# piotrkawa/audio-deepfake-adversarial-attacks

Measured on AMD Instinct MI355X. Metric: adversarial utterances/sec, PGD-40 LCNN+LFCC 4s@16kHz, higher is better.
Workload: dtype f32

## Files before the change

### audio_deepfake_adversarial_attacks_amd/csrc/lfcc_stft.hip

```cpp

#include <hip/hip_runtime.h>
#include <math.h>
#include <stdint.h>
#include <stdlib.h>

#include "advstep_frontend.h"
#include "advstep_common.h"
#include "stft_reg.h"

namespace {

constexpr int kWavesPerBlock = 4;
constexpr int kThreads = kWavesPerBlock * 64;
constexpr int kFramesPerBlockBwd = 4;
static_assert(kFramesPerBlockBwd == kGroup, "overlap_add_frames (stft_reg.h) sums the frames of one group");

__device__ __forceinline__ float2 cmul(float2 a, float2 b) { return make_float2(a.x * b.x - a.y * b.y, a.x * b.y + a.y * b.x); }

__device__ __forceinline__ void wave_lds_sync() {
    __builtin_amdgcn_fence(__ATOMIC_RELEASE, "workgroup");
    __builtin_amdgcn_wave_barrier();
    __builtin_amdgcn_fence(__ATOMIC_ACQUIRE, "workgroup");
}

// ... 132 lines not shown
    __syncthreads();
    if (threadIdx.x == 0) {
        float r = L.red[0];
        for (int i = 1; i < kWavesPerBlock; ++i) r = max_nan(r, L.red[i]);
        bmax[b * gridDim.x + blockIdx.x] = r;
    }
}

constexpr int kMaxSpanT = 8, kMaxBands = 128;

__device__ __forceinline__ void frame_spectrum(const float *__restrict__ xb, const float *__restrict__ w, int T, int f,
                                               int hop, Lds &L, int wave, int lane) {
    load_frame(xb, w, T, f, hop, L.a[wave], lane);
    wave_lds_sync();
    fft256<false>(L.a[wave], L.b[wave], L.tw, lane);
    unpack_real(L.a[wave], L.tw512, L.xs_of(wave), lane);
    wave_lds_sync();
}

__device__ __forceinline__ float2 one_sided_scale(float2 gk, int k) {
    if (k == 0 || k == kN) gk.y = 0.0f;
    else gk.x *= 0.5f, gk.y *= 0.5f;
    return gk;
}

template <bool PRESCALED>
__device__ __forceinline__ void spectrum_grad_to_frame(Lds &L, int wave, int lane, const float *__restrict__ w, float *dst,
                                                       bool live) {
    if (!PRESCALED) {
        for (int k = lane; k < kBins; k += 64) L.xs_of(wave)[k] = one_sided_scale(L.xs_of(wave)[k], k);
        wave_lds_sync();
    }
    for (int k = lane; k < kN; k += 64) {
        const float2 gk = L.xs_of(wave)[k], gc = conjf2(L.xs_of(wave)[kN - k]);
        const float2 e = cadd(gk, gc), d = csub(gk, gc);
        const float2 wd = cmul(conjf2(L.tw512[k]), d);
        L.a[wave][P(k)] = make_float2(e.x - wd.y, e.y + wd.x);
    }
    wave_lds_sync();
    fft256<true>(L.a[wave], L.b[wave], L.tw, lane);
    for (int n = lane; n < kN; n += 64) {
        const float2 z = L.a[wave][P(n)];
        const float2 wv = reinterpret_cast<const float2 *>(w)[n];
        reinterpret_cast<float2 *>(dst)[n] = live ? make_float2(wv.x * z.x, wv.y * z.y) : make_float2(0.0f, 0.0f);
    }
    wave_lds_sync();
}

template <int STRIDE>
__device__ __attribute__((noinline)) void overlap_add_frames_cold(const float *dframe, float *__restrict__ dxb, int f_base, int NF, int hop,
                                                                  int T, int tid, int nthreads);

__device__ __forceinline__ void overlap_add_block(const float (*dframe)[kNfft], float *__restrict__ dxb, int f_base, int NF,
                                                  int hop, int T) {
    overlap_add_frames<kNfft>(&dframe[0][0], dxb, f_base, NF, hop, T, threadIdx.x, kThreads);
}

template <int STRIDE>
__device__ __attribute__((noinline)) void overlap_add_frames_cold(const float *dframe, float *__restrict__ dxb, int f_base, int NF, int hop,
                                                                  int T, int tid, int nthreads) {
    overlap_add_frames<STRIDE>(dframe, dxb, f_base, NF, hop, T, tid, nthreads);
}

template <int SPAN_CAP>
struct LdsBwd {
    Lds c;
    float dframe[kFramesPerBlockBwd][kNfft];
    float fbt_w[kBins * SPAN_CAP];
    int32_t fbt_start[kBins];
    float drow[kWavesPerBlock][kMaxBands];
};

template <int SPAN_CAP>
__global__ __launch_bounds__(kThreads) void stft_bands_backward_kernel(const float *__restrict__ x,
                                                                       const float *__restrict__ w,
                                                                       const float *__restrict__ dband,
                                                                       const int32_t *__restrict__ fbt_start,
                                                                       const float *__restrict__ fbt_w, int span_t,
                                                                       float *__restrict__ dx, int T, int NF, int hop,
                                                                       int M) {
    extern __shared__ __attribute__((aligned(16))) unsigned char raw[];
    LdsBwd<SPAN_CAP> &S = *reinterpret_cast<LdsBwd<SPAN_CAP> *>(raw);
    Lds &L = S.c;
    {
        static_assert(kN == kThreads, "one twiddle pair per thread");
        constexpr int kWIt = (kBins * SPAN_CAP + kThreads - 1) / kThreads;
        const int m = threadIdx.x, nw = kBins * span_t;
        const float2 t0 = stage_twiddle(m < kStageTw ? m : 0), t1 = kTw512[m];
        const int32_t s0 = fbt_start[m], s1 = fbt_start[kThreads + (m < kBins - kThreads ? m : 0)];
        float wq[kWIt];
#pragma unroll
        for (int j = 0; j < kWIt; ++j) {
            const int i = m + j * kThreads;
            wq[j] = fbt_w[i < nw ? i : nw - 1];
        }
        if (m < kStageTw) L.tw[m] = t0;
        L.tw512[m] = t1;
        S.fbt_start[m] = s0;
        if (m < kBins - kThreads) S.fbt_start[kThreads + m] = s1;
#pragma unroll
        for (int j = 0; j < kWIt; ++j) {
            const int i = m + j * kThreads;
            if (i < nw) S.fbt_w[i] = wq[j];
        }
    }
    __syncthreads();
    const int wave = threadIdx.x >> 6, lane = threadIdx.x & 63;
    const int64_t b = blockIdx.y;
    const int f_base = blockIdx.x * kFramesPerBlockBwd;
    const float *xb = x + b * T;
    for (int r = 0; r < kFramesPerBlockBwd / kWavesPerBlock; ++r) {
        const int fl = r * kWavesPerBlock + wave;
        const int f = f_base + fl;
        const bool live = f < NF;
        const float *drow_g = dband + (b * NF + (live ? f : NF - 1)) * M;
        for (int m = lane; m < M; m += 64) S.drow[wave][m] = drow_g[m];
        load_frame(xb, w, T, live ? f : NF - 1, hop, L.a[wave], lane);
        wave_lds_sync();
        fft256<false>(L.a[wave], L.b[wave], L.tw, lane);
        const float *drow = S.drow[wave];
        auto grad_of_bin = [&](int k, float2 xk) {
            const int m0 = S.fbt_start[k];
            float dp = 0.0f;
            for (int j = 0; j < span_t; ++j) {
                const int m = m0 + j;
                if (m < M) dp = fmaf(S.fbt_w[k * span_t + j], drow[m], dp);
            }
            return one_sided_scale(make_float2(2.0f * xk.x * dp, 2.0f * xk.y * dp), k);
        };
        {
            const float2 *Z = L.a[wave];
            for (int k = lane; k < kN; k += 64) {
                const float2 zk = Z[P(k)], zc = conjf2(Z[P((kN - k) & (kN - 1))]);
                const float2 e = make_float2(0.5f * (zk.x + zc.x), 0.5f * (zk.y + zc.y));
                const float2 d = make_float2(0.5f * (zk.x - zc.x), 0.5f * (zk.y - zc.y));
                const float2 o = cmul(L.tw512[k], make_float2(d.y, -d.x));
                L.xs_of(wave)[k] = grad_of_bin(k, cadd(e, o));
            }
            if (lane == 0) L.xs_of(wave)[kN] = grad_of_bin(kN, make_float2(Z[P(0)].x - Z[P(0)].y, 0.0f));
        }
        wave_lds_sync();
        spectrum_grad_to_frame<true>(L, wave, lane, w, S.dframe[fl], live);
    }
    __syncthreads();
    overlap_add_block(S.dframe, dx + b * T, f_base, NF, hop, T);
}

#ifndef STFT_FWD_GROUPS
#define STFT_FWD_GROUPS 2
#endif
constexpr int kGroupsPerWave = STFT_FWD_GROUPS;
constexpr int kBandsFramesPerBlock = kWavesPerBlock * kGroupsPerWave * kGroup;

struct LdsReg {
    float2 blk[kWavesPerBlock][kGroup][kFrameSlots];
    float2 twl[16 * kPitch];
    float red[kWavesPerBlock];
};

__device__ __forceinline__ void fill_reg_tables(LdsReg &S) {
    for (int m = threadIdx.x; m < kN; m += kThreads) S.twl[(m >> 4) * kPitch + (m & 15)] = kTw256[((m >> 4) * (m & 15)) & 255];
}

__device__ __forceinline__ void load_frame_reg(const float *__restrict__ xb, const float2 *__restrict__ win2, int T, int f, int hop,
                                               float2 (&x)[16], int l) {
    const int q_first = f * hop - kN;
    if (q_first >= 0 && q_first + kNfft <= T && ((q_first & 1) == 0) && ((reinterpret_cast<uintptr_t>(xb) & 7u) == 0)) {
        const float2 *x2 = reinterpret_cast<const float2 *>(xb + q_first);
        float2 v[16];
#pragma unroll
        for (int r = 0; r < 16; ++r) v[r] = x2[16 * r + l];
#pragma unroll
        for (int r = 0; r < 16; ++r) {
            const float2 wv = win2[16 * r + l];
            x[r] = make_float2(wv.x * v[r].x, wv.y * v[r].y);
        }
        return;
    }
#pragma unroll
    for (int r = 0; r < 16; ++r) {
        const int n = 16 * r + l;
        int q0 = q_first + 2 * n, q1 = q0 + 1;
        q0 = q0 < 0 ? -q0 : q0;
        q0 = q0 >= T ? 2 * (T - 1) - q0 : q0;
        q1 = q1 < 0 ? -q1 : q1;
        q1 = q1 >= T ? 2 * (T - 1) - q1 : q1;
        const float2 wv = win2[n];
        x[r] = make_float2(wv.x * xb[q0], wv.y * xb[q1]);
    }
}

constexpr int kRegSpan = 4;

struct LdsRegFwd {
    LdsReg c;
    float fbw[kMaxBands * kRegSpan];
    int32_t fbs[kMaxBands];
};

__global__ __launch_bounds__(kThreads) void stft_bands_reg_kernel(const float *__restrict__ x, const float *__restrict__ w,
                                                                  const int32_t *__restrict__ fb_start,
                                                                  const float *__restrict__ fb_w, int span,
                                                                  float *__restrict__ band_db, float *__restrict__ bmax, int T,
                                                                  int NF, int hop, int M, int bmax_tail) {
    __shared__ LdsRegFwd SF;
    LdsReg &S = SF.c;
    fill_reg_tables(S);
    for (int i = threadIdx.x; i < kMaxBands * kRegSpan; i += kThreads) {
        const int m = i / kRegSpan, j = i % kRegSpan;
        SF.fbw[i] = (m < M && j < span) ? 0.25f * fb_w[m * span + j] : 0.0f;
    }
    for (int m = threadIdx.x; m < kMaxBands; m += kThreads) SF.fbs[m] = m < M ? fb_start[m] : 0;
    const int wave = threadIdx.x >> 6, lane = threadIdx.x & 63, fs = lane >> 4, l = lane & 15;
    __syncthreads();
    const int64_t b = blockIdx.y;
    float2 *blk = S.blk[wave][fs];
    float vmax = -INFINITY;
    for (int g = 0; g < kGroupsPerWave; ++g) {
        const int f0 = blockIdx.x * kBandsFramesPerBlock + (wave * kGroupsPerWave + g) * kGroup;
        if (f0 >= NF) break;
        const int f = f0 + fs;
        const bool live = f < NF;
        float2 xr[16];
        load_frame_reg(x + b * T, reinterpret_cast<const float2 *>(w), T, live ? f : NF - 1, hop, xr, here(l));
        fft256_reg<false>(xr, S.twl, blk, l);
        float nyq;
        unpack_real_reg(xr, nyq, blk, l);
        phase_done(xr);
        float *pw = reinterpret_cast<float *>(blk);
        lds_wave_fence();
#pragma unroll
        for (int r = 0; r < 16; ++r) pw[l + 16 * r] = fmaf(xr[r].x, xr[r].x, xr[r].y * xr[r].y);
        if (l == 0) pw[kN] = nyq * nyq;
        if (l >= 1 && l <= kRegSpan) pw[kN + l] = 0.0f;
        lds_wave_fence();
        float *row = band_db + (b * NF + (live ? f : NF - 1)) * M;
#pragma unroll
        for (int half = 0; half < 2; ++half) {
            int k0[4];
            float wt[4][kRegSpan], pv[4][kRegSpan];
#pragma unroll
            for (int i = 0; i < 4; ++i) k0[i] = SF.fbs[l + 16 * (4 * half + i)];
#pragma unroll
            for (int i = 0; i < 4; ++i)
#pragma unroll
                for (int j = 0; j < kRegSpan; ++j) {
                    wt[i][j] = SF.fbw[(l + 16 * (4 * half + i)) * kRegSpan + j];
                    pv[i][j] = pw[k0[i] + j];
                }
#pragma unroll
            for (int i = 0; i < 4; ++i) {
                const int m = l + 16 * (4 * half + i);
                float band = 0.0f;
#pragma unroll
                for (int j = 0; j < kRegSpan; ++j) band = fmaf(wt[i][j], pv[i][j], band);
                const float db = 3.010299956639812f * __log2f(band > kAmin ? band : (band != band ? band : kAmin));
                if (live && m < M) {
                    row[m] = db;
                    vmax = max_nan(vmax, db);
                }
            }
        }
        lds_wave_fence();
    }
    vmax = wave_reduce(vmax, MaxNanOp());
    if (lane == 0) S.red[wave] = vmax;
    __syncthreads();
    if (threadIdx.x == 0) {
        float r = S.red[0];
        for (int i = 1; i < kWavesPerBlock; ++i) r = max_nan(r, S.red[i]);
        bmax[b * gridDim.x + blockIdx.x] = r;
        const int total = gridDim.x * gridDim.y;
        for (int j = (int)b * gridDim.x + blockIdx.x; j < bmax_tail; j += total) bmax[total + j] = -INFINITY;
    }
}

template <int STRIDE>
__device__ __forceinline__ void overlap_add_interior(const float *df, float *__restrict__ out, int lane, float (&carry)[6],
                                                     bool carry_in, bool carry_out) {
    constexpr int HOP = 160, kSpan = 3 * HOP + kNfft, kShared = kNfft - HOP;
    static_assert(4 * HOP == 640 && kSpan <= 16 * 64, "slices");
#pragma unroll
    for (int j = 0; j < 16; ++j) {
        if (j % 4 == 0) lds_wave_fence();
        float acc = 0.0f;
#pragma unroll
        for (int fl = 0; fl < 4; ++fl) {
            const int lo = HOP * fl - 64 * j, hi = lo + kNfft;
            if (hi <= 0 || lo >= 64) continue;
            if (lo <= 0 && hi >= 64) {
                acc += df[fl * STRIDE + lane - lo];
            } else {
                const int n = lane - lo;
                if ((unsigned)n < (unsigned)kNfft) acc += df[fl * STRIDE + n];
            }
        }
        const int i = lane + 64 * j;
        if (j < 6) {
            const bool shared = i < kShared;
            if (carry_in) {
                out[i] = shared ? acc + carry[j] : acc;
            } else if (j < 5) {
                atomicAdd(out + i, acc);
            } else {
                if (shared) atomicAdd(out + i, acc);
                else out[i] = acc;
            }
        } else if (j < 10) {
            out[i] = acc;
        } else {
            if (carry_out) carry[j - 10] = acc;
            else if (i < kSpan) atomicAdd(out + i, acc);
        }
    }
}

template <int SPAN_CAP>
struct LdsRegBwd {
    LdsReg c;
    float fbt_w[(kBins + 1) * SPAN_CAP];
    int32_t fbt_start[kBins + 1];
};

#ifndef STFT_BWD_GROUPS
#define STFT_BWD_GROUPS 4
#endif
constexpr int kBwdGroupsPerWave = STFT_BWD_GROUPS;
constexpr int kBwdFramesPerBlock = kWavesPerBlock * kBwdGroupsPerWave * kGroup;

#ifndef STFT_BWD_WAVES
#define STFT_BWD_WAVES 4
#endif
template <int SPAN_CAP>
__global__ __launch_bounds__(kThreads) __attribute__((amdgpu_waves_per_eu(STFT_BWD_WAVES, STFT_BWD_WAVES)))
void stft_bands_backward_reg_kernel(const float *__restrict__ x,
                                                                           const float *__restrict__ w,
                                                                           const float *__restrict__ dband,
                                                                           const int32_t *__restrict__ fbt_start,
                                                                           const float *__restrict__ fbt_w, int span_t,
                                                                           float *__restrict__ dx, int T, int NF, int hop,
                                                                           int M, const float *__restrict__ band_db,
                                                                           const float *__restrict__ stats) {
    extern __shared__ __attribute__((aligned(16))) unsigned char raw[];
    LdsRegBwd<SPAN_CAP> &S = *reinterpret_cast<LdsRegBwd<SPAN_CAP> *>(raw);
    float fix_share = 0.0f, fix_max = 0.0f;
    bool fix = false;
    if (stats != nullptr) {
        const float s2 = stats[2];
        if (s2 != 0.0f) {
            fix = true;
            fix_max = stats[0];
            fix_share = s2 / (stats[1] > 0.0f ? stats[1] : 1.0f);
        }
    }
    fill_reg_tables(S.c);
    for (int i = threadIdx.x; i < kBins * SPAN_CAP; i += kThreads) {
        const int k = i / SPAN_CAP, j = i % SPAN_CAP;
        S.fbt_w[i] = j < span_t ? fbt_w[k * span_t + j] : 0.0f;
    }
    for (int i = threadIdx.x; i < kBins; i += kThreads) S.fbt_start[i] = fbt_start[i];
    const int wave = threadIdx.x >> 6, lane = threadIdx.x & 63, fs = lane >> 4, l = lane & 15;
    __syncthreads();
    const int64_t b = blockIdx.y;
    const float *xb = x + b * T;
    float2 *blk = S.c.blk[wave][fs];
    float carry[6] = {0.0f, 0.0f, 0.0f, 0.0f, 0.0f, 0.0f};
    bool carried = false;
    auto interior = [&](int g0) {
        return hop == 160 && g0 + kGroup <= NF && g0 * hop >= 2 * kN && g0 * hop + 3 * hop + kNfft <= T;
    };
    for (int g = 0; g < kBwdGroupsPerWave; ++g) {
        const int f0 = blockIdx.x * kBwdFramesPerBlock + (wave * kBwdGroupsPerWave + g) * kGroup;
        if (f0 >= NF) break;
        const int f = f0 + fs;
        const bool live = f < NF;
        const int fc = live ? f : NF - 1;
        float dreg[kMaxBands / 16];
        {
            const float *src = dband + (b * NF + fc) * M;
#pragma unroll
            for (int i = 0; i < kMaxBands / 16; ++i) {
                const int m = l + 16 * i;
                dreg[i] = m < M ? src[m] : 0.0f;
            }
            if (fix) {
                const float *dbrow = band_db + (b * NF + fc) * M;
#pragma unroll
                for (int i = 0; i < kMaxBands / 16; ++i) {
                    const int m = l + 16 * i;
                    const float db = m < M ? dbrow[m] : 0.0f;
                    if (m < M && db == fix_max) dreg[i] += fix_share * dlog_of_db(db);
                }
            }
        }
        float2 xr[16];
        load_frame_reg(xb, reinterpret_cast<const float2 *>(w), T, fc, hop, xr, here(l));
        phase_done(xr);
        fft256_reg<false>(xr, S.c.twl, blk, l);
        float nyq;
        unpack_real_reg(xr, nyq, blk, l);
        phase_done(xr);
        float *drow = reinterpret_cast<float *>(blk);
        lds_wave_fence();
#pragma unroll
        for (int i = 0; i < kMaxBands / 16; ++i) drow[l + 16 * i] = dreg[i];
        if (l < SPAN_CAP) drow[kMaxBands + l] = 0.0f;
#pragma unroll
        for (int q = 0; q < 4; ++q) {
            lds_wave_fence();
            int m0[4];
#pragma unroll
            for (int i = 0; i < 4; ++i) m0[i] = S.fbt_start[l + 16 * (4 * q + i)];
#pragma unroll
            for (int i = 0; i < 4; ++i) {
                const int r = 4 * q + i;
                float dp = 0.0f;
#pragma unroll
                for (int j = 0; j < SPAN_CAP; ++j) dp = fmaf(S.fbt_w[(l + 16 * r) * SPAN_CAP + j], drow[m0[i] + j], dp);
                const bool dc = r == 0 && l == 0;
                const float c = dc ? dp : 0.5f * dp;
                xr[r] = make_float2(c * xr[r].x, dc ? 0.0f : c * xr[r].y);
            }
            asm volatile("" : "+v"(xr[4 * q].x), "+v"(xr[4 * q].y), "+v"(xr[4 * q + 1].x), "+v"(xr[4 * q + 1].y), "+v"(xr[4 * q + 2].x),
                              "+v"(xr[4 * q + 2].y), "+v"(xr[4 * q + 3].x), "+v"(xr[4 * q + 3].y) :: "memory");
        }
        float g_nyq = 0.0f;
        if (l == 0) {
            const int m0n = S.fbt_start[kN];
            float dpn = 0.0f;
#pragma unroll
            for (int j = 0; j < SPAN_CAP; ++j) dpn = fmaf(S.fbt_w[kN * SPAN_CAP + j], drow[m0n + j], dpn);
            g_nyq = dpn * nyq;
        }
        phase_done(xr);
        lds_wave_fence();
        park_vector(blk, xr, l);
        lds_wave_fence();
        int lp = here(l);
#pragma unroll
        for (int r = 0; r < 16; ++r) {
            if (r == 8) half_done<0>(xr);
            float2 gc = conjf2(mirror_of(blk, r, l));
            if (r == 0 && l == 0) gc = make_float2(g_nyq, 0.0f);
            const float2 e = cadd(xr[r], gc), d = csub(xr[r], gc);
            const float2 wd = cmulf(conjf2(kTw512[lp + 16 * r]), d);
            xr[r] = make_float2(e.x - wd.y, e.y + wd.x);
        }
        fft256_reg<true>(xr, S.c.twl, blk, l);
        lds_wave_fence();
        lp = here(l);
#pragma unroll
        for (int r = 0; r < 16; ++r) {
            const float2 wv = reinterpret_cast<const float2 *>(w)[lp + 16 * r];
            blk[l + 16 * r] = live ? make_float2(wv.x * xr[r].x, wv.y * xr[r].y) : make_float2(0.0f, 0.0f);
        }
        lds_wave_fence();
        const float *df = reinterpret_cast<const float *>(S.c.blk[wave][0]);
        if (interior(f0)) {
            const bool carry_out = g + 1 < kBwdGroupsPerWave && f0 + kGroup < NF && interior(f0 + kGroup);
            overlap_add_interior<2 * kFrameSlots>(df, dx + b * T + (f0 * hop - kN), lane, carry, carried, carry_out);
            carried = carry_out;
        } else {
            overlap_add_frames_cold<2 * kFrameSlots>(df, dx + b * T, f0, NF, hop, T, lane, 64);
            carried = false;
        }
        lds_wave_fence();
    }
}

constexpr int kMelMax = 80;
constexpr int kMelMaxSpan = 48;

struct LdsMel {
    Lds c;
    float2 y[kWavesPerBlock][kMelMax];
    float stage[2][kMelMax][kFramesPerBlockFwd + 1];
};

template <int CAP>
struct MelTaps {
    float w[2][CAP];
    int f0[2];
};

template <int CAP>
__device__ __forceinline__ void load_mel_taps(MelTaps<CAP> &t, int lane, const int32_t *__restrict__ fb_start,
                                              const float *__restrict__ fb_w, int span, int M) {
#pragma unroll
    for (int pass = 0; pass < 2; ++pass) {
        const int m = lane + 64 * pass;
        const bool live = m < M;
        const int f0 = live ? fb_start[m] : 0;
        t.f0[pass] = f0;
#pragma unroll
        for (int j = 0; j < CAP; ++j) t.w[pass][j] = (live && j < span && f0 + j < kBins) ? fb_w[m * span + j] : 0.0f;
    }
}

template <int CAP>
__device__ __forceinline__ void mel_bands(const Lds &L, int wave, int lane, const MelTaps<CAP> &t, int M, float2 *y) {
#pragma unroll
    for (int pass = 0; pass < 2; ++pass) {
        const int m = lane + 64 * pass;
        if (m < M) {
            float re = 0.0f, im = 0.0f;
#pragma unroll
            for (int j = 0; j < CAP; ++j) {
                const int k = t.f0[pass] + j < kBins ? t.f0[pass] + j : kBins - 1;
                const float2 z = L.xs_of(wave)[k];
                re = fmaf(t.w[pass][j], z.x, re);
                im = fmaf(t.w[pass][j], z.y, im);
            }
            y[m] = make_float2(re, im);
        }
    }
}

template <int CAP>
__global__ __launch_bounds__(kThreads) void stft_mel_kernel(const float *__restrict__ x, const float *__restrict__ w,
                                                            const int32_t *__restrict__ fb_start,
                                                            const float *__restrict__ fb_w, int span,
                                                            float *__restrict__ out, int T, int NF, int hop, int M) {
    extern __shared__ __attribute__((aligned(16))) unsigned char raw[];
    LdsMel &S = *reinterpret_cast<LdsMel *>(raw);
    Lds &L = S.c;
    fill_twiddles(L);
    __syncthreads();
    const int wave = threadIdx.x >> 6, lane = threadIdx.x & 63;
    const int64_t b = blockIdx.y;
    const int f_base = blockIdx.x * kFramesPerBlockFwd;
    MelTaps<CAP> taps;
    load_mel_taps(taps, lane, fb_start, fb_w, span, M);
    for (int r = 0; r < kFramesPerBlockFwd / kWavesPerBlock; ++r) {
        const int fl = r * kWavesPerBlock + wave, f = f_base + fl;
        if (f >= NF) break;
        frame_spectrum(x + b * T, w, T, f, hop, L, wave, lane);
        mel_bands(L, wave, lane, taps, M, S.y[wave]);
        wave_lds_sync();
        for (int m = lane; m < M; m += 64) {
            const float2 v = S.y[wave][m];
            S.stage[0][m][fl] = sqrtf(v.x * v.x + v.y * v.y);
            S.stage[1][m][fl] = atan2f(v.y, v.x);
        }
        wave_lds_sync();
    }
    __syncthreads();
    const int frames_here = (NF - f_base) < kFramesPerBlockFwd ? (NF - f_base) : kFramesPerBlockFwd;
    for (int i = threadIdx.x; i < 2 * M * kFramesPerBlockFwd; i += kThreads) {
        const int fl = i % kFramesPerBlockFwd, row = i / kFramesPerBlockFwd, plane = row / M, m = row - plane * M;
        if (fl < frames_here) out[((b * 2 + plane) * M + m) * NF + f_base + fl] = S.stage[plane][m][fl];
    }
}

struct LdsMelBwd {
    Lds c;
    float dframe[kFramesPerBlockBwd][kNfft];
    float2 y[kWavesPerBlock][kMelMax];
    float stage[2][kMelMax][kFramesPerBlockBwd + 1];
};

template <int CAP, int SPT>
__global__ __launch_bounds__(kThreads) void stft_mel_backward_kernel(const float *__restrict__ x, const float *__restrict__ w,
                                                                     const float *__restrict__ dout,
                                                                     const int32_t *__restrict__ fb_start,
                                                                     const float *__restrict__ fb_w, int span,
                                                                     const int32_t *__restrict__ fbt_start,
                                                                     const float *__restrict__ fbt_w, int span_t,
                                                                     float *__restrict__ dx, int T, int NF, int hop, int M) {
    extern __shared__ __attribute__((aligned(16))) unsigned char raw[];
    LdsMelBwd &S = *reinterpret_cast<LdsMelBwd *>(raw);
    Lds &L = S.c;
    fill_twiddles(L);
    const int wave = threadIdx.x >> 6, lane = threadIdx.x & 63;
    const int64_t b = blockIdx.y;
    const int f_base = blockIdx.x * kFramesPerBlockBwd;
    const int frames_here = (NF - f_base) < kFramesPerBlockBwd ? (NF - f_base) : kFramesPerBlockBwd;
    for (int i = threadIdx.x; i < 2 * M * kFramesPerBlockBwd; i += kThreads) {
        const int fl = i % kFramesPerBlockBwd, row = i / kFramesPerBlockBwd, plane = row / M, m = row - plane * M;
        S.stage[plane][m][fl] = fl < frames_here ? dout[((b * 2 + plane) * M + m) * NF + f_base + fl] : 0.0f;
    }
    __syncthreads();
    const float *xb = x + b * T;
    MelTaps<CAP> taps;
    load_mel_taps(taps, lane, fb_start, fb_w, span, M);
    constexpr int kBinPasses = (kBins + 63) / 64;
    float tw_t[kBinPasses][SPT];
    int m0_t[kBinPasses];
#pragma unroll
    for (int p = 0; p < kBinPasses; ++p) {
        const int k = lane + 64 * p;
        const bool in = k < kBins;
        m0_t[p] = in ? fbt_start[k] : 0;
#pragma unroll
        for (int j = 0; j < SPT; ++j) tw_t[p][j] = (in && j < span_t && m0_t[p] + j < M) ? fbt_w[k * span_t + j] : 0.0f;
    }
    for (int r = 0; r < kFramesPerBlockBwd / kWavesPerBlock; ++r) {
        const int fl = r * kWavesPerBlock + wave, f = f_base + fl;
        const bool live = f < NF;
        frame_spectrum(xb, w, T, live ? f : NF - 1, hop, L, wave, lane);
        mel_bands(L, wave, lane, taps, M, S.y[wave]);
        wave_lds_sync();
        for (int m = lane; m < M; m += 64) {
            const float2 v = S.y[wave][m];
            const float gm = S.stage[0][m][fl], gp = S.stage[1][m][fl];
            const float n2 = v.x * v.x + v.y * v.y;
            float2 gy = make_float2(0.0f, 0.0f);
            if (n2 > 0.0f) {
// ... 188 lines not shown
                tile[(1 * kMelMax + m) * (kBandsFramesPerBlock + 1) + fl] = ph[g][i];
            }
        }
    }
    __syncthreads();
    const int frames_here = (NF - f_base) < kBandsFramesPerBlock ? (NF - f_base) : kBandsFramesPerBlock;
    for (int i = threadIdx.x; i < 2 * M * kBandsFramesPerBlock; i += kThreads) {
        const int fl = i % kBandsFramesPerBlock, row = i / kBandsFramesPerBlock, plane = row / M, m = row - plane * M;
        if (fl < frames_here)
            out[((b * 2 + plane) * M + m) * NF + f_base + fl] = tile[(plane * kMelMax + m) * (kBandsFramesPerBlock + 1) + fl];
    }
}

template <int SPAN_CAP>
struct LdsMelRegBwd {
    LdsReg c;
    float fbt_w[(kBins + 1) * SPAN_CAP];
    int32_t fbt_start[kBins + 1];
};

template <int SPAN_CAP>
__global__ __launch_bounds__(kThreads) void stft_mel_backward_out_reg_kernel(const float *__restrict__ w, const float *__restrict__ dout,
                                                                             const float *__restrict__ out,
                                                                             const int32_t *__restrict__ fbt_start,
                                                                             const float *__restrict__ fbt_w, int span_t,
                                                                             float *__restrict__ dx, int T, int NF, int hop, int M) {
    extern __shared__ __attribute__((aligned(16))) unsigned char raw[];
    LdsMelRegBwd<SPAN_CAP> &S = *reinterpret_cast<LdsMelRegBwd<SPAN_CAP> *>(raw);
    fill_reg_tables(S.c);
    for (int i = threadIdx.x; i < kBins * SPAN_CAP; i += kThreads) {
        const int k = i / SPAN_CAP, j = i % SPAN_CAP;
        S.fbt_w[i] = j < span_t ? fbt_w[k * span_t + j] : 0.0f;
    }
    for (int i = threadIdx.x; i < kBins; i += kThreads) S.fbt_start[i] = fbt_start[i];
    const int wave = threadIdx.x >> 6, lane = threadIdx.x & 63, fs = lane >> 4, l = lane & 15;
    __syncthreads();
    const int64_t b = blockIdx.y;
    float2 *blk = S.c.blk[wave][fs];
    float carry[6] = {0.0f, 0.0f, 0.0f, 0.0f, 0.0f, 0.0f};
    bool carried = false;
    auto interior = [&](int g0) {
        return hop == 160 && g0 + kGroup <= NF && g0 * hop >= 2 * kN && g0 * hop + 3 * hop + kNfft <= T;
    };
    constexpr int kRows = 4 * kMelMax;
    static_assert((kRows + 2 * (kMelMax + 8)) * sizeof(float) <= kFrameSlots * sizeof(float2), "stage + d Y fit a frame's block");
    for (int g = 0; g < kBwdGroupsPerWave; ++g) {
        const int f0 = blockIdx.x * kBwdFramesPerBlock + (wave * kBwdGroupsPerWave + g) * kGroup;
        if (f0 >= NF) break;
        const int f = f0 + fs;
        const bool live = f < NF;
        float *stage = reinterpret_cast<float *>(blk);
        {
            float *wave_blocks = reinterpret_cast<float *>(S.c.blk[wave][0]);
            for (int i = lane; i < 4 * M * kGroup; i += 64) {
                const int fl = i & 3, row = i >> 2, plane = row / M, m = row - plane * M;
                const float *src = plane < 2 ? dout : out;
                const float v = f0 + fl < NF ? src[((b * 2 + (plane & 1)) * M + m) * NF + f0 + fl] : 0.0f;
                wave_blocks[fl * 2 * kFrameSlots + plane * kMelMax + m] = v;
            }
        }
        lds_wave_fence();
        float2 *dy = reinterpret_cast<float2 *>(stage + kRows);
#pragma unroll
        for (int i = 0; i < kMelBandsPerLane; ++i) {
            const int m = l + 16 * i;
            if (m < kMelMax) {
                float2 gy = make_float2(0.0f, 0.0f);
                if (m < M) {
                    const float gm = stage[m], gp = stage[kMelMax + m], mg = stage[2 * kMelMax + m], phv = stage[3 * kMelMax + m];
                    if (mg > 0.0f) {
                        float sn, cs;
                        sincosf(phv, &sn, &cs);
                        const float q = gp / mg;
                        gy.x = gm * cs - q * sn;
                        gy.y = gm * sn + q * cs;
                    }
                }
                dy[m] = gy;
            }
        }
        if (l < 8) dy[kMelMax + l] = make_float2(0.0f, 0.0f);
        lds_wave_fence();
        float2 xr[16];
#pragma unroll
        for (int q = 0; q < 4; ++q) {
            lds_wave_fence();
            int m0[4];
#pragma unroll
            for (int i = 0; i < 4; ++i) m0[i] = S.fbt_start[l + 16 * (4 * q + i)];
#pragma unroll
            for (int i = 0; i < 4; ++i) {
                const int r = 4 * q + i;
                float re = 0.0f, im = 0.0f;
#pragma unroll
                for (int j = 0; j < SPAN_CAP; ++j) {
                    const float wt = S.fbt_w[(l + 16 * r) * SPAN_CAP + j];
                    const float2 gy = dy[m0[i] + j];
                    re = fmaf(wt, gy.x, re);
                    im = fmaf(wt, gy.y, im);
                }
                const bool dc = r == 0 && l == 0;
                xr[r] = dc ? make_float2(re, 0.0f) : make_float2(0.5f * re, 0.5f * im);
            }
            asm volatile("" : "+v"(xr[4 * q].x), "+v"(xr[4 * q].y), "+v"(xr[4 * q + 1].x), "+v"(xr[4 * q + 1].y), "+v"(xr[4 * q + 2].x),
                              "+v"(xr[4 * q + 2].y), "+v"(xr[4 * q + 3].x), "+v"(xr[4 * q + 3].y) :: "memory");
        }
        float g_nyq = 0.0f;
        if (l == 0) {
            const int m0n = S.fbt_start[kN];
#pragma unroll
            for (int j = 0; j < SPAN_CAP; ++j) g_nyq = fmaf(S.fbt_w[kN * SPAN_CAP + j], dy[m0n + j].x, g_nyq);
        }
        phase_done(xr);
        lds_wave_fence();
        park_vector(blk, xr, l);
        lds_wave_fence();
        int lp = here(l);
#pragma unroll
        for (int r = 0; r < 16; ++r) {
            if (r == 8) half_done<0>(xr);
            float2 gc = conjf2(mirror_of(blk, r, l));
            if (r == 0 && l == 0) gc = make_float2(g_nyq, 0.0f);
            const float2 e = cadd(xr[r], gc), d = csub(xr[r], gc);
            const float2 wd = cmulf(conjf2(kTw512[lp + 16 * r]), d);
            xr[r] = make_float2(e.x - wd.y, e.y + wd.x);
        }
        fft256_reg<true>(xr, S.c.twl, blk, l);
        lds_wave_fence();
        lp = here(l);
#pragma unroll
        for (int r = 0; r < 16; ++r) {
            const float2 wv = reinterpret_cast<const float2 *>(w)[lp + 16 * r];
            blk[l + 16 * r] = live ? make_float2(wv.x * xr[r].x, wv.y * xr[r].y) : make_float2(0.0f, 0.0f);
        }
        lds_wave_fence();
        const float *df = reinterpret_cast<const float *>(S.c.blk[wave][0]);
        if (interior(f0)) {
            const bool carry_out = g + 1 < kBwdGroupsPerWave && f0 + kGroup < NF && interior(f0 + kGroup);
            overlap_add_interior<2 * kFrameSlots>(df, dx + b * T + (f0 * hop - kN), lane, carry, carried, carry_out);
            carried = carry_out;
        } else {
            overlap_add_frames_cold<2 * kFrameSlots>(df, dx + b * T, f0, NF, hop, T, lane, 64);
            carried = false;
        }
        lds_wave_fence();
    }
}

inline bool reg_fft_enabled() {
    const char *e = getenv("ADVSTEP_STFT_REG");
    return !(e && e[0] == '0');
}

int stft_bands_backward_launch(const float *x, const float *window, const float *dband, const int32_t *fbt_start, const float *fbt_w,
                               int64_t span_t, float *dx, int64_t B, int64_t T, int64_t NF, int64_t hop, int64_t nfft, int64_t M,
                               const float *band_db, const float *stats, int dx_is_zero, advstep_stream_t stream) {
    ADVSTEP_REQUIRE(B >= 0 && NF >= 0 && M >= 0 && span_t >= 1);
    if (B == 0 || T == 0) return ADVSTEP_OK;
    ADVSTEP_REQUIRE(x && window && dband && fbt_start && fbt_w && dx && B <= kMaxGridY);
    ADVSTEP_REQUIRE(advstep_stft_bands_supported(nfft, hop, T) && NF == 1 + T / hop && span_t <= kMaxSpanT && M <= kMaxBands);
    ADVSTEP_REQUIRE(kFramesPerBlockBwd * hop >= kNfft - hop);
    hipStream_t st = as_stream(stream);
    if (!dx_is_zero && hipMemsetAsync(dx, 0, (size_t)B * T * sizeof(float), st) != hipSuccess) return ADVSTEP_ELAUNCH;
    const bool reg = reg_fft_enabled();
    const dim3 grid((unsigned)ceil_div(NF, reg ? kBwdFramesPerBlock : kFramesPerBlockBwd), (unsigned)B);
    if (reg) {
        auto go = [&](auto kernel, size_t lds) {
            (void)hipFuncSetAttribute(reinterpret_cast<const void *>(kernel), hipFuncAttributeMaxDynamicSharedMemorySize, (int)lds);
            hipLaunchKernelGGL(kernel, grid, dim3(kThreads), lds, st, x, window, dband, fbt_start, fbt_w, (int)span_t, dx, (int)T,
                               (int)NF, (int)hop, (int)M, band_db, stats);
        };
        if (span_t <= 2) go(stft_bands_backward_reg_kernel<2>, sizeof(LdsRegBwd<2>));
        else go(stft_bands_backward_reg_kernel<kMaxSpanT>, sizeof(LdsRegBwd<kMaxSpanT>));
    } else {
        auto go = [&](auto kernel, size_t lds) {
            (void)hipFuncSetAttribute(reinterpret_cast<const void *>(kernel), hipFuncAttributeMaxDynamicSharedMemorySize, (int)lds);
            hipLaunchKernelGGL(kernel, grid, dim3(kThreads), lds, st, x, window, dband, fbt_start, fbt_w, (int)span_t, dx, (int)T,
                               (int)NF, (int)hop, (int)M);
        };
        if (span_t <= 2) go(stft_bands_backward_kernel<2>, sizeof(LdsBwd<2>));
        else go(stft_bands_backward_kernel<kMaxSpanT>, sizeof(LdsBwd<kMaxSpanT>));
    }
    return status_after_launch();
}
}

extern "C" {

size_t advstep_stft_bands_block_count(int64_t B, int64_t NF) {
    if (B <= 0 || NF <= 0) return 0;
    return (size_t)(B * ceil_div(NF, kFramesPerBlockFwd));
}

int advstep_stft_bands_supported(int64_t nfft, int64_t hop, int64_t T) {
    return nfft == kNfft && hop >= 128 && hop <= kNfft && T > kN + 1;
}

int advstep_stft_bands_f32(const float *x, const float *window, const int32_t *fb_start, const float *fb_w, int64_t span,
                           float *band_db, float *block_max, int64_t B, int64_t T, int64_t NF, int64_t hop, int64_t nfft,
                           int64_t M, advstep_stream_t stream) {
    ADVSTEP_REQUIRE(B >= 0 && NF >= 0 && M >= 0 && span >= 1);
    if (B == 0 || NF == 0 || M == 0) return ADVSTEP_OK;
    ADVSTEP_REQUIRE(x && window && fb_start && fb_w && band_db && block_max && B <= kMaxGridY);
    ADVSTEP_REQUIRE(advstep_stft_bands_supported(nfft, hop, T) && NF == 1 + T / hop);
    if (reg_fft_enabled() && span <= kRegSpan && M <= kMaxBands) {
        const int64_t blocks32 = ceil_div(NF, kBandsFramesPerBlock), blocks16 = ceil_div(NF, kFramesPerBlockFwd);
        ADVSTEP_REQUIRE(B * blocks16 <= INT32_MAX);
        const dim3 grid((unsigned)blocks32, (unsigned)B);
        hipLaunchKernelGGL(stft_bands_reg_kernel, grid, dim3(kThreads), 0, as_stream(stream), x, window, fb_start, fb_w, (int)span,
                           band_db, block_max, (int)T, (int)NF, (int)hop, (int)M, (int)(B * (blocks16 - blocks32)));
        return status_after_launch();
    }
    const dim3 grid((unsigned)ceil_div(NF, kFramesPerBlockFwd), (unsigned)B);
    hipLaunchKernelGGL(stft_bands_kernel, grid, dim3(kThreads), 0, as_stream(stream), x, window, fb_start, fb_w, (int)span,
                       band_db, block_max, (int)T, (int)NF, (int)hop, (int)M);
    return status_after_launch();
}

int advstep_stft_bands_backward_f32(const float *x, const float *window, const float *dband, const int32_t *fbt_start,
                                    const float *fbt_w, int64_t span_t, float *dx, int64_t B, int64_t T, int64_t NF,
                                    int64_t hop, int64_t nfft, int64_t M, advstep_stream_t stream) {
    return stft_bands_backward_launch(x, window, dband, fbt_start, fbt_w, span_t, dx, B, T, NF, hop, nfft, M, nullptr, nullptr, 0,
                                      stream);
}

int advstep_stft_bands_backward_fixup_f32(const float *x, const float *window, float *dband, const float *band_db,
                                          const float *stats, const int32_t *fbt_start, const float *fbt_w, int64_t span_t,
                                          float *dx, int dx_is_zero, int64_t B, int64_t T, int64_t NF, int64_t hop,
                                          int64_t nfft, int64_t M, advstep_stream_t stream) {
    ADVSTEP_REQUIRE(band_db && stats);
    if (!reg_fft_enabled()) {
        if (B > 0 && NF > 0 && M > 0) {
            const int st = advstep_lfcc_floor_fixup_f32(band_db, stats, dband, B * NF * M, stream);
            if (st != ADVSTEP_OK) return st;
        }
        return stft_bands_backward_launch(x, window, dband, fbt_start, fbt_w, span_t, dx, B, T, NF, hop, nfft, M, nullptr, nullptr,
                                          dx_is_zero, stream);
    }
    return stft_bands_backward_launch(x, window, dband, fbt_start, fbt_w, span_t, dx, B, T, NF, hop, nfft, M, band_db, stats,
                                      dx_is_zero, stream);
}

int advstep_stft_mel_f32(const float *x, const float *window, const int32_t *fb_start, const float *fb_w, int64_t span,
                         float *out, int64_t B, int64_t T, int64_t NF, int64_t hop, int64_t nfft, int64_t M,
                         advstep_stream_t stream) {
    ADVSTEP_REQUIRE(B >= 0 && NF >= 0 && M >= 0 && span >= 1);
    if (B == 0 || NF == 0 || M == 0) return ADVSTEP_OK;
    ADVSTEP_REQUIRE(x && window && fb_start && fb_w && out && B <= kMaxGridY && M <= kMelMax && span <= kMelMaxSpan);
    ADVSTEP_REQUIRE(advstep_stft_bands_supported(nfft, hop, T) && NF == 1 + T / hop);
    hipStream_t st = as_stream(stream);
    if (reg_fft_enabled() && span <= kMelRegSpan) {
        const size_t lds_reg = sizeof(LdsMelReg);
        (void)hipFuncSetAttribute(reinterpret_cast<const void *>(stft_mel_reg_kernel), hipFuncAttributeMaxDynamicSharedMemorySize,
                                  (int)lds_reg);
        hipLaunchKernelGGL(stft_mel_reg_kernel, dim3((unsigned)ceil_div(NF, kBandsFramesPerBlock), (unsigned)B), dim3(kThreads),
                           lds_reg, st, x, window, fb_start, fb_w, (int)span, out, (int)T, (int)NF, (int)hop, (int)M);
        return status_after_launch();
    }
    const size_t lds = sizeof(LdsMel);
    auto go = [&](auto kernel) {
        (void)hipFuncSetAttribute(reinterpret_cast<const void *>(kernel), hipFuncAttributeMaxDynamicSharedMemorySize, (int)lds);
        hipLaunchKernelGGL(kernel, dim3((unsigned)ceil_div(NF, kFramesPerBlockFwd), (unsigned)B), dim3(kThreads), lds, st, x,
                           window, fb_start, fb_w, (int)span, out, (int)T, (int)NF, (int)hop, (int)M);
    };
    if (span <= 16) go(stft_mel_kernel<16>);
    else go(stft_mel_kernel<kMelMaxSpan>);
    return status_after_launch();
}

int advstep_stft_mel_backward_f32(const float *x, const float *window, const float *dout, const int32_t *fb_start,
                                  const float *fb_w, int64_t span, const int32_t *fbt_start, const float *fbt_w,
                                  int64_t span_t, float *dx, int64_t B, int64_t T, int64_t NF, int64_t hop, int64_t nfft,
                                  int64_t M, advstep_stream_t stream) {
    ADVSTEP_REQUIRE(B >= 0 && NF >= 0 && M >= 0 && span >= 1 && span_t >= 1);
    if (B == 0 || T == 0) return ADVSTEP_OK;
    ADVSTEP_REQUIRE(x && window && dout && fb_start && fb_w && fbt_start && fbt_w && dx && B <= kMaxGridY && M <= kMelMax &&
                    span <= kMelMaxSpan && span_t <= kMaxSpanT);
    ADVSTEP_REQUIRE(advstep_stft_bands_supported(nfft, hop, T) && NF == 1 + T / hop);
    ADVSTEP_REQUIRE(kFramesPerBlockBwd * hop >= kNfft - hop);
    hipStream_t st = as_stream(stream);
    if (hipMemsetAsync(dx, 0, (size_t)B * T * sizeof(float), st) != hipSuccess) return ADVSTEP_ELAUNCH;
    const size_t lds = sizeof(LdsMelBwd);
    auto go = [&](auto kernel) {
        (void)hipFuncSetAttribute(reinterpret_cast<const void *>(kernel), hipFuncAttributeMaxDynamicSharedMemorySize, (int)lds);
        hipLaunchKernelGGL(kernel, dim3((unsigned)ceil_div(NF, kFramesPerBlockBwd), (unsigned)B), dim3(kThreads), lds, st, x,
                           window, dout, fb_start, fb_w, (int)span, fbt_start, fbt_w, (int)span_t, dx, (int)T, (int)NF, (int)hop,
                           (int)M);
    };
    if (span <= 16 && span_t <= 2) go(stft_mel_backward_kernel<16, 2>);
    else if (span_t <= 2) go(stft_mel_backward_kernel<kMelMaxSpan, 2>);
    else go(stft_mel_backward_kernel<kMelMaxSpan, kMaxSpanT>);
    return status_after_launch();
}

int advstep_stft_mel_backward_from_output_f32(const float *window, const float *dout, const float *out, const int32_t *fbt_start,
                                              const float *fbt_w, int64_t span_t, float *dx, int64_t B, int64_t T, int64_t NF,
                                              int64_t hop, int64_t nfft, int64_t M, advstep_stream_t stream) {
    ADVSTEP_REQUIRE(B >= 0 && NF >= 0 && M >= 0 && span_t >= 1);
    if (B == 0 || T == 0) return ADVSTEP_OK;
    ADVSTEP_REQUIRE(window && dout && out && fbt_start && fbt_w && dx && B <= kMaxGridY && M <= kMelMax && span_t <= kMaxSpanT);
    ADVSTEP_REQUIRE(advstep_stft_bands_supported(nfft, hop, T) && NF == 1 + T / hop);
    ADVSTEP_REQUIRE(kFramesPerBlockBwd * hop >= kNfft - hop);
    hipStream_t st = as_stream(stream);
    if (hipMemsetAsync(dx, 0, (size_t)B * T * sizeof(float), st) != hipSuccess) return ADVSTEP_ELAUNCH;
    if (reg_fft_enabled()) {
        auto go_reg = [&](auto kernel, size_t lds_reg) {
            (void)hipFuncSetAttribute(reinterpret_cast<const void *>(kernel), hipFuncAttributeMaxDynamicSharedMemorySize, (int)lds_reg);
            hipLaunchKernelGGL(kernel, dim3((unsigned)ceil_div(NF, kBwdFramesPerBlock), (unsigned)B), dim3(kThreads), lds_reg, st, window,
                               dout, out, fbt_start, fbt_w, (int)span_t, dx, (int)T, (int)NF, (int)hop, (int)M);
        };
        if (span_t <= 2) go_reg(stft_mel_backward_out_reg_kernel<2>, sizeof(LdsMelRegBwd<2>));
        else go_reg(stft_mel_backward_out_reg_kernel<kMaxSpanT>, sizeof(LdsMelRegBwd<kMaxSpanT>));
        return status_after_launch();
    }
    const size_t lds = sizeof(LdsMelBwdOut);
    auto go = [&](auto kernel) {
        (void)hipFuncSetAttribute(reinterpret_cast<const void *>(kernel), hipFuncAttributeMaxDynamicSharedMemorySize, (int)lds);
        hipLaunchKernelGGL(kernel, dim3((unsigned)ceil_div(NF, kFramesPerBlockBwd), (unsigned)B), dim3(kThreads), lds, st, window,
                           dout, out, fbt_start, fbt_w, (int)span_t, dx, (int)T, (int)NF, (int)hop, (int)M);
    };
    if (span_t <= 2) go(stft_mel_backward_out_kernel<2>);
    else go(stft_mel_backward_out_kernel<kMaxSpanT>);
    return status_after_launch();
}

}
// ... 1 lines not shown
```

### audio_deepfake_adversarial_attacks_amd/csrc/stft_reg.h

```cpp

#ifndef ADVSTEP_STFT_REG_H
#define ADVSTEP_STFT_REG_H

#include <hip/hip_runtime.h>
#include <stdint.h>

#include "advstep_common.h"

namespace {

constexpr int kN = 256;
constexpr int kNfft = 2 * kN;
constexpr int kBins = kN + 1;
constexpr int kGroup = 4;
constexpr int kPitch = 17;
constexpr int kFrameSlots = 16 * kPitch;

__device__ __forceinline__ float2 cadd(float2 a, float2 b) { return make_float2(a.x + b.x, a.y + b.y); }
__device__ __forceinline__ float2 csub(float2 a, float2 b) { return make_float2(a.x - b.x, a.y - b.y); }
__device__ __forceinline__ float2 conjf2(float2 a) { return make_float2(a.x, -a.y); }

#include "stft_tables.inc"

__device__ __forceinline__ float2 cmulf(float2 a, float2 b) {
    return make_float2(fmaf(a.x, b.x, -(a.y * b.y)), fmaf(a.x, b.y, a.y * b.x));
}
__device__ __forceinline__ float2 cmulc(float2 a, float cr, float ci) { return cmulf(a, make_float2(cr, ci)); }

template <bool INV>
__device__ __forceinline__ void fft4(float2 &a, float2 &b, float2 &c, float2 &d) {
    const float2 s02 = cadd(a, c), d02 = csub(a, c), s13 = cadd(b, d), d13 = csub(b, d);
    const float2 r = INV ? make_float2(-d13.y, d13.x) : make_float2(d13.y, -d13.x);
    a = cadd(s02, s13);
    b = cadd(d02, r);
    c = csub(s02, s13);
    d = csub(d02, r);
}

template <bool INV>
__device__ __forceinline__ void fft16(float2 (&x)[16]) {
    constexpr float C1 = 0.92387953251128674f, S1 = 0.38268343236508977f, H = 0.70710678118654752f;
#pragma unroll
    for (int n2 = 0; n2 < 4; ++n2) fft4<INV>(x[n2], x[4 + n2], x[8 + n2], x[12 + n2]);
    const float sg = INV ? 1.0f : -1.0f;
    x[4 + 1] = cmulc(x[4 + 1], C1, sg * S1);
    x[8 + 1] = cmulc(x[8 + 1], H, sg * H);
    x[12 + 1] = cmulc(x[12 + 1], S1, sg * C1);
    x[4 + 2] = cmulc(x[4 + 2], H, sg * H);
    x[8 + 2] = INV ? make_float2(-x[8 + 2].y, x[8 + 2].x) : make_float2(x[8 + 2].y, -x[8 + 2].x);
    x[12 + 2] = cmulc(x[12 + 2], -H, sg * H);
    x[4 + 3] = cmulc(x[4 + 3], S1, sg * C1);
    x[8 + 3] = cmulc(x[8 + 3], -H, sg * H);
    x[12 + 3] = cmulc(x[12 + 3], -C1, -sg * S1);
#pragma unroll
    for (int k1 = 0; k1 < 4; ++k1) fft4<INV>(x[4 * k1], x[4 * k1 + 1], x[4 * k1 + 2], x[4 * k1 + 3]);
#pragma unroll
    for (int i = 0; i < 4; ++i)
#pragma unroll
        for (int j = i + 1; j < 4; ++j) {
            const float2 t = x[4 * i + j];
            x[4 * i + j] = x[4 * j + i];
            x[4 * j + i] = t;
        }
}

__device__ __forceinline__ int here(int v) {
    asm volatile("" : "+v"(v));
    return v;
}

__device__ __forceinline__ void phase_done(float2 (&x)[16]) {
    asm volatile("" : "+v"(x[0].x), "+v"(x[0].y), "+v"(x[1].x), "+v"(x[1].y), "+v"(x[2].x), "+v"(x[2].y), "+v"(x[3].x), "+v"(x[3].y),
                      "+v"(x[4].x), "+v"(x[4].y), "+v"(x[5].x), "+v"(x[5].y), "+v"(x[6].x), "+v"(x[6].y), "+v"(x[7].x), "+v"(x[7].y)
                 :: "memory");
    asm volatile("" : "+v"(x[8].x), "+v"(x[8].y), "+v"(x[9].x), "+v"(x[9].y), "+v"(x[10].x), "+v"(x[10].y), "+v"(x[11].x), "+v"(x[11].y),
                      "+v"(x[12].x), "+v"(x[12].y), "+v"(x[13].x), "+v"(x[13].y), "+v"(x[14].x), "+v"(x[14].y), "+v"(x[15].x), "+v"(x[15].y)
                 :: "memory");
}

template <int BASE>
__device__ __forceinline__ void half_done(float2 (&x)[16]) {
    asm volatile("" : "+v"(x[BASE].x), "+v"(x[BASE].y), "+v"(x[BASE + 1].x), "+v"(x[BASE + 1].y), "+v"(x[BASE + 2].x), "+v"(x[BASE + 2].y),
                      "+v"(x[BASE + 3].x), "+v"(x[BASE + 3].y), "+v"(x[BASE + 4].x), "+v"(x[BASE + 4].y), "+v"(x[BASE + 5].x),
                      "+v"(x[BASE + 5].y), "+v"(x[BASE + 6].x), "+v"(x[BASE + 6].y), "+v"(x[BASE + 7].x), "+v"(x[BASE + 7].y)
                 :: "memory");
}

__device__ __forceinline__ void lds_wave_fence() { asm volatile("s_waitcnt lgkmcnt(0)" ::: "memory"); }

__device__ __forceinline__ void fill_twiddle_rows(float2 *twl) {
    for (int m = threadIdx.x; m < kN; m += blockDim.x) twl[(m >> 4) * kPitch + (m & 15)] = kTw256[((m >> 4) * (m & 15)) & 255];
}

template <bool INV>
__device__ __forceinline__ void fft256_reg(float2 (&x)[16], const float2 *twl, float2 *blk, int l) {
    fft16<INV>(x);
    phase_done(x);
#pragma unroll
    for (int j = 1; j < 16; ++j) {
        const float2 t = twl[l * kPitch + j];
        x[j] = cmulf(x[j], INV ? conjf2(t) : t);
    }
    lds_wave_fence();
#pragma unroll
    for (int j = 0; j < 16; ++j) blk[j * kPitch + l] = x[j];
    lds_wave_fence();
#pragma unroll
    for (int j = 0; j < 16; ++j) x[j] = blk[l * kPitch + j];
    fft16<INV>(x);
}

__device__ __forceinline__ void park_vector(float2 *blk, const float2 (&x)[16], int l) {
#pragma unroll
    for (int r = 0; r < 16; ++r) blk[r * kPitch + l] = x[r];
    if (l == 0) {
#pragma unroll
        for (int r = 0; r < 16; ++r) blk[((r + 15) & 15) * kPitch + 16] = x[r];
    }
}
__device__ __forceinline__ float2 mirror_of(const float2 *blk, int r, int l) { return blk[(15 - r) * kPitch + (16 - l)]; }

__device__ __forceinline__ void unpack_real_reg(float2 (&x)[16], float &nyq, float2 *blk, int l) {
    lds_wave_fence();
    park_vector(blk, x, l);
    lds_wave_fence();
    nyq = 2.0f * (x[0].x - x[0].y);
    const int lt = here(l);
#pragma unroll
    for (int r = 0; r < 16; ++r) {
        if (r == 8) half_done<0>(x);
        const float2 zc = conjf2(mirror_of(blk, r, l));
        const float2 e = cadd(x[r], zc), d = csub(x[r], zc);
        x[r] = cadd(e, cmulf(kTw512[lt + 16 * r], make_float2(d.y, -d.x)));
    }
}

__device__ __forceinline__ void pack_real_reg(float2 (&x)[16], float g_nyq, float2 *blk, int l) {
    phase_done(x);
    lds_wave_fence();
    park_vector(blk, x, l);
    lds_wave_fence();
    const int lp = here(l);
#pragma unroll
    for (int r = 0; r < 16; ++r) {
        if (r == 8) half_done<0>(x);
        float2 gc = conjf2(mirror_of(blk, r, l));
        if (r == 0 && l == 0) gc = make_float2(g_nyq, 0.0f);
        const float2 e = cadd(x[r], gc), d = csub(x[r], gc);
        const float2 wd = cmulf(conjf2(kTw512[lp + 16 * r]), d);
        x[r] = make_float2(e.x - wd.y, e.y + wd.x);
    }
}

template <int STRIDE>
__device__ __forceinline__ void overlap_add_frames(const float *dframe, float *__restrict__ dxb, int f_base, int NF, int hop, int T,
                                                   int tid, int nthreads) {
    const int p_lo = f_base * hop;
    const int frames_here = (NF - f_base) < kGroup ? (NF - f_base) : kGroup;
    const int p_hi = p_lo + (frames_here - 1) * hop + kNfft;
    auto add_from = [&](int p, float &acc) {
        if (p < p_lo || p >= p_hi) return;
#pragma unroll
        for (int fl = 0; fl < kGroup; ++fl) {
            const int n = p - p_lo - fl * hop;
            if (fl < frames_here && n >= 0 && n < kNfft) acc += dframe[fl * STRIDE + n];
        }
    };
    const bool near_left = p_lo < 2 * kN, near_right = p_hi > T;
    const int t_first = p_lo - kN, span_all = p_hi - p_lo;
    for (int i = tid; i < span_all; i += nthreads) {
        const int t = t_first + i;
        if (t < 0 || t >= T) continue;
        float acc = 0.0f;
        add_from(t + kN, acc);
        if (near_left && t >= 1 && t <= kN) add_from(kN - t, acc);
        if (near_right && t <= T - 2 && t >= T - 1 - kN) add_from(2 * (T - 1) - t + kN, acc);
        if (acc != 0.0f) atomicAdd(dxb + t, acc);
    }
    if (!(near_left || near_right)) return;
    for (int i = tid; i < span_all; i += nthreads) {
        const int p = p_lo + i, q = p - kN;
        int t = -1;
        if (q < 0) t = -q;
        else if (q >= T) t = 2 * (T - 1) - q;
        if (t < 0 || t >= T) continue;
        const int pd = t + kN;
        if (pd >= p_lo && pd < p_hi) continue;
        float acc = 0.0f;
        add_from(p, acc);
        if (acc != 0.0f) atomicAdd(dxb + t, acc);
    }
}

}

#endif
```

Baseline: 2103.

## Stage window and twiddle tables in LDS with 8-wave backward STFT blocks

Adds a variant of the register-FFT STFT backward kernel that copies the analysis window and the 512-point twiddle table into LDS once per block and reads them from there. The block size doubles to 8 waves, so the staging cost is shared across more frames. The variant is used by default when span_t<=2 and can be turned off with an environment variable. Launch failures from the LDS attribute now return an error. The larger LDS footprint and larger blocks may lower occupancy, and calls to fill_twiddle_rows rely on a helper not shown.

After: 2108 (median of 2 runs). No clear change (+0.2%).

```diff
diff --git a/audio_deepfake_adversarial_attacks_amd/csrc/lfcc_stft.hip b/audio_deepfake_adversarial_attacks_amd/csrc/lfcc_stft.hip
--- a/audio_deepfake_adversarial_attacks_amd/csrc/lfcc_stft.hip
+++ b/audio_deepfake_adversarial_attacks_amd/csrc/lfcc_stft.hip
@@ -308,11 +308,32 @@
 constexpr int kGroupsPerWave = STFT_FWD_GROUPS;
 constexpr int kBandsFramesPerBlock = kWavesPerBlock * kGroupsPerWave * kGroup;
 
-struct LdsReg {
-    float2 blk[kWavesPerBlock][kGroup][kFrameSlots];
+template <int WAVES>
+struct LdsRegW {
+    float2 blk[WAVES][kGroup][kFrameSlots];
     float2 twl[16 * kPitch];
-    float red[kWavesPerBlock];
+    float red[WAVES];
 };
+using LdsReg = LdsRegW<kWavesPerBlock>;
+
+template <bool LT>
+struct RegLayout {
+    static constexpr int kWaves = LT ? 2 * kWavesPerBlock : kWavesPerBlock;
+    static constexpr int kThreads = 64 * kWaves;
+};
+template <bool LT>
+struct StagedTables {};
+template <>
+struct StagedTables<true> {
+    float2 win2[kN];
+    float2 w512[kN];
+};
+__device__ __forceinline__ void stage_tables(StagedTables<true> &t, const float *__restrict__ w) {
+    for (int m = threadIdx.x; m < kN; m += blockDim.x) {
+        t.win2[m] = reinterpret_cast<const float2 *>(w)[m];
+        t.w512[m] = kTw512[m];
+    }
+}
 
 __device__ __forceinline__ void fill_reg_tables(LdsReg &S) {
     for (int m = threadIdx.x; m < kN; m += kThreads) S.twl[(m >> 4) * kPitch + (m & 15)] = kTw256[((m >> 4) * (m & 15)) & 255];
@@ -471,11 +492,12 @@
     }
 }
 
-template <int SPAN_CAP>
+template <int SPAN_CAP, bool LT = false>
 struct LdsRegBwd {
-    LdsReg c;
+    LdsRegW<RegLayout<LT>::kWaves> c;
     float fbt_w[(kBins + 1) * SPAN_CAP];
     int32_t fbt_start[kBins + 1];
+    StagedTables<LT> t;
 };
 
 #ifndef STFT_BWD_GROUPS
@@ -483,12 +505,20 @@
 #endif
 constexpr int kBwdGroupsPerWave = STFT_BWD_GROUPS;
 constexpr int kBwdFramesPerBlock = kWavesPerBlock * kBwdGroupsPerWave * kGroup;
+#ifndef STFT_BWD_GROUPS_LDS
+#define STFT_BWD_GROUPS_LDS 4
+#endif
+template <bool LT>
+struct BwdLayout : RegLayout<LT> {
+    static constexpr int kGroups = LT ? STFT_BWD_GROUPS_LDS : kBwdGroupsPerWave;
+    static constexpr int kFramesPerBlock = RegLayout<LT>::kWaves * kGroups * kGroup;
+};
 
 #ifndef STFT_BWD_WAVES
 #define STFT_BWD_WAVES 4
 #endif
-template <int SPAN_CAP>
-__global__ __launch_bounds__(kThreads) __attribute__((amdgpu_waves_per_eu(STFT_BWD_WAVES, STFT_BWD_WAVES)))
+template <int SPAN_CAP, bool LT>
+__global__ __launch_bounds__(RegLayout<LT>::kThreads) __attribute__((amdgpu_waves_per_eu(STFT_BWD_WAVES, STFT_BWD_WAVES)))
 void stft_bands_backward_reg_kernel(const float *__restrict__ x,
                                                                            const float *__restrict__ w,
                                                                            const float *__restrict__ dband,
@@ -497,8 +527,10 @@
                                                                            float *__restrict__ dx, int T, int NF, int hop,
                                                                            int M, const float *__restrict__ band_db,
                                                                            const float *__restrict__ stats) {
+    using Lay = BwdLayout<LT>;
+    constexpr int kThreads = Lay::kThreads, kBwdGroupsPerWave = Lay::kGroups, kBwdFramesPerBlock = Lay::kFramesPerBlock;
     extern __shared__ __attribute__((aligned(16))) unsigned char raw[];
-    LdsRegBwd<SPAN_CAP> &S = *reinterpret_cast<LdsRegBwd<SPAN_CAP> *>(raw);
+    LdsRegBwd<SPAN_CAP, LT> &S = *reinterpret_cast<LdsRegBwd<SPAN_CAP, LT> *>(raw);
     float fix_share = 0.0f, fix_max = 0.0f;
     bool fix = false;
     if (stats != nullptr) {
@@ -509,12 +541,19 @@
             fix_share = s2 / (stats[1] > 0.0f ? stats[1] : 1.0f);
         }
     }
-    fill_reg_tables(S.c);
+    fill_twiddle_rows(S.c.twl);
     for (int i = threadIdx.x; i < kBins * SPAN_CAP; i += kThreads) {
         const int k = i / SPAN_CAP, j = i % SPAN_CAP;
         S.fbt_w[i] = j < span_t ? fbt_w[k * span_t + j] : 0.0f;
     }
     for (int i = threadIdx.x; i < kBins; i += kThreads) S.fbt_start[i] = fbt_start[i];
+    const float2 *win2, *w512;
+    if constexpr (LT) {
+        stage_tables(S.t, w);
+        win2 = S.t.win2, w512 = S.t.w512;
+    } else {
+        win2 = reinterpret_cast<const float2 *>(w), w512 = kTw512;
+    }
     const int wave = threadIdx.x >> 6, lane = threadIdx.x & 63, fs = lane >> 4, l = lane & 15;
     __syncthreads();
     const int64_t b = blockIdx.y;
@@ -550,11 +589,11 @@
             }
         }
         float2 xr[16];
-        load_frame_reg(xb, reinterpret_cast<const float2 *>(w), T, fc, hop, xr, here(l));
+        load_frame_reg(xb, win2, T, fc, hop, xr, here(l));
         phase_done(xr);
         fft256_reg<false>(xr, S.c.twl, blk, l);
         float nyq;
-        unpack_real_reg(xr, nyq, blk, l);
+        unpack_real_reg(xr, nyq, blk, l, TablePtr{w512});
         phase_done(xr);
         float *drow = reinterpret_cast<float *>(blk);
         lds_wave_fence();
@@ -599,16 +638,22 @@
             float2 gc = conjf2(mirror_of(blk, r, l));
             if (r == 0 && l == 0) gc = make_float2(g_nyq, 0.0f);
             const float2 e = cadd(xr[r], gc), d = csub(xr[r], gc);
-            const float2 wd = cmulf(conjf2(kTw512[lp + 16 * r]), d);
+            const float2 wd = cmulf(conjf2(w512[lp + 16 * r]), d);
             xr[r] = make_float2(e.x - wd.y, e.y + wd.x);
         }
         fft256_reg<true>(xr, S.c.twl, blk, l);
         lds_wave_fence();
         lp = here(l);
 #pragma unroll
-        for (int r = 0; r < 16; ++r) {
-            const float2 wv = reinterpret_cast<const float2 *>(w)[lp + 16 * r];
-            blk[l + 16 * r] = live ? make_float2(wv.x * xr[r].x, wv.y * xr[r].y) : make_float2(0.0f, 0.0f);
+        for (int h = 0; h < 2; ++h) {
+            float2 wv[8];
+#pragma unroll
+            for (int i = 0; i < 8; ++i) wv[i] = win2[lp + 16 * (8 * h + i)];
+#pragma unroll
+            for (int i = 0; i < 8; ++i) {
+                const int r = 8 * h + i;
+                blk[l + 16 * r] = live ? make_float2(wv[i].x * xr[r].x, wv[i].y * xr[r].y) : make_float2(0.0f, 0.0f);
+            }
         }
         lds_wave_fence();
         const float *df = reinterpret_cast<const float *>(S.c.blk[wave][0]);
@@ -1103,6 +1148,16 @@
     return !(e && e[0] == '0');
 }
 
+inline bool stft_tables_in_lds() {
+    const char *e = getenv("ADVSTEP_STFT_TABLES");
+    return !(e && e[0] == 'g');
+}
+
+template <class K>
+inline bool allow_lds(K kernel, size_t lds) {
+    return hipFuncSetAttribute(reinterpret_cast<const void *>(kernel), hipFuncAttributeMaxDynamicSharedMemorySize, (int)lds) == hipSuccess;
+}
+
 int stft_bands_backward_launch(const float *x, const float *window, const float *dband, const int32_t *fbt_start, const float *fbt_w,
                                int64_t span_t, float *dx, int64_t B, int64_t T, int64_t NF, int64_t hop, int64_t nfft, int64_t M,
                                const float *band_db, const float *stats, int dx_is_zero, advstep_stream_t stream) {
@@ -1114,15 +1169,21 @@
     hipStream_t st = as_stream(stream);
     if (!dx_is_zero && hipMemsetAsync(dx, 0, (size_t)B * T * sizeof(float), st) != hipSuccess) return ADVSTEP_ELAUNCH;
     const bool reg = reg_fft_enabled();
-    const dim3 grid((unsigned)ceil_div(NF, reg ? kBwdFramesPerBlock : kFramesPerBlockBwd), (unsigned)B);
+    const bool lt = reg && span_t <= 2 && stft_tables_in_lds();
+    const dim3 grid((unsigned)ceil_div(NF, lt ? BwdLayout<true>::kFramesPerBlock : reg ? kBwdFramesPerBlock : kFramesPerBlockBwd),
+                    (unsigned)B);
     if (reg) {
-        auto go = [&](auto kernel, size_t lds) {
-            (void)hipFuncSetAttribute(reinterpret_cast<const void *>(kernel), hipFuncAttributeMaxDynamicSharedMemorySize, (int)lds);
-            hipLaunchKernelGGL(kernel, grid, dim3(kThreads), lds, st, x, window, dband, fbt_start, fbt_w, (int)span_t, dx, (int)T,
+        auto go = [&](auto kernel, size_t lds, int threads) {
+            if (!allow_lds(kernel, lds)) return false;
+            hipLaunchKernelGGL(kernel, grid, dim3(threads), lds, st, x, window, dband, fbt_start, fbt_w, (int)span_t, dx, (int)T,
                                (int)NF, (int)hop, (int)M, band_db, stats);
+            return true;
         };
-        if (span_t <= 2) go(stft_bands_backward_reg_kernel<2>, sizeof(LdsRegBwd<2>));
-        else go(stft_bands_backward_reg_kernel<kMaxSpanT>, sizeof(LdsRegBwd<kMaxSpanT>));
+        bool ok;
+        if (lt) ok = go(stft_bands_backward_reg_kernel<2, true>, sizeof(LdsRegBwd<2, true>), BwdLayout<true>::kThreads);
+        else if (span_t <= 2) ok = go(stft_bands_backward_reg_kernel<2, false>, sizeof(LdsRegBwd<2>), kThreads);
+        else ok = go(stft_bands_backward_reg_kernel<kMaxSpanT, false>, sizeof(LdsRegBwd<kMaxSpanT>), kThreads);
+        if (!ok) return ADVSTEP_ELAUNCH;
     } else {
         auto go = [&](auto kernel, size_t lds) {
             (void)hipFuncSetAttribute(reinterpret_cast<const void *>(kernel), hipFuncAttributeMaxDynamicSharedMemorySize, (int)lds);
diff --git a/audio_deepfake_adversarial_attacks_amd/csrc/stft_reg.h b/audio_deepfake_adversarial_attacks_amd/csrc/stft_reg.h
--- a/audio_deepfake_adversarial_attacks_amd/csrc/stft_reg.h
+++ b/audio_deepfake_adversarial_attacks_amd/csrc/stft_reg.h
@@ -120,7 +120,16 @@
 }
 __device__ __forceinline__ float2 mirror_of(const float2 *blk, int r, int l) { return blk[(15 - r) * kPitch + (16 - l)]; }
 
-__device__ __forceinline__ void unpack_real_reg(float2 (&x)[16], float &nyq, float2 *blk, int l) {
+struct Tw512Global {
+    __device__ __forceinline__ float2 operator()(int k) const { return kTw512[k]; }
+};
+struct TablePtr {
+    const float2 *p;
+    __device__ __forceinline__ float2 operator()(int k) const { return p[k]; }
+};
+
+template <class TW>
+__device__ __forceinline__ void unpack_real_reg(float2 (&x)[16], float &nyq, float2 *blk, int l, TW tw512) {
     lds_wave_fence();
     park_vector(blk, x, l);
     lds_wave_fence();
@@ -131,8 +140,11 @@
         if (r == 8) half_done<0>(x);
         const float2 zc = conjf2(mirror_of(blk, r, l));
         const float2 e = cadd(x[r], zc), d = csub(x[r], zc);
-        x[r] = cadd(e, cmulf(kTw512[lt + 16 * r], make_float2(d.y, -d.x)));
-    }
+        x[r] = cadd(e, cmulf(tw512(lt + 16 * r), make_float2(d.y, -d.x)));
+    }
+}
+__device__ __forceinline__ void unpack_real_reg(float2 (&x)[16], float &nyq, float2 *blk, int l) {
+    unpack_real_reg(x, nyq, blk, l, Tw512Global());
 }
 
 __device__ __forceinline__ void pack_real_reg(float2 (&x)[16], float g_nyq, float2 *blk, int l) {
```
